# pirovc/ganon

Measured on AMD Instinct MI355X. Metric: Mreads/s classified (150 bp) + IBF-lookup GB/s vs HBM roofline, higher is better.
Workload: dtype u64

## Files before the change

ganon_amd/csrc/gn_kernels.hip:

```cpp
#include "gn_internal.h"
#include <cstdlib>

#define GN_WAVE 64
#define GN_CAND_LIMIT 128u
#ifndef GN_NARROW_MAX
#define GN_NARROW_MAX 4u
#endif
#include "gn_stray_probe.h"
static_assert(GN_PROBE_HASHES % 2u == 0 && GN_PROBE_HASHES * 4u <= GN_WAVE, "whole screen iterations (two hashes each), and stage 1 is one load a lane");
#define GN_MATCH_CHUNK 256u
#ifndef GN_MATCH_CHUNK_MAX
#define GN_MATCH_CHUNK_MAX 8192u
#endif
#define GN_STAGE_CAP 128u

struct GnRankLut
{
    uint8_t t[256];
    constexpr GnRankLut() : t{}
    {
        for (int i = 0; i < 256; ++i)
            t[i] = 0;
        t['C'] = t['c'] = 1;
        t['G'] = t['g'] = 2;
// ... 1434 lines not shown
                        q_to    = n;
                    }
                    const uint32_t inc  = add << (8u * (bit >> 3));
                    const uint32_t keep = SCR && finish ? ~(0xFFu << (8u * (bit >> 3))) : 0xFFFFFFFFu;
#pragma unroll
                    for (int j = 0; j < 4; ++j)
#pragma unroll
                        for (int pp = 0; pp < 2; ++pp)
                            if ((bit & 3u) == (uint32_t)j && ((bit >> 2) & 1u) == (uint32_t)pp && lane == L)
                                byt[d][j][pp] = (byt[d][j][pp] & keep) + inc;
                }
            }
        }
    }
    if (slice * 64 * LW < p.W)
    {
        const uint32_t wcol = p.W - slice * 64 * LW < 64u * LW ? p.W - slice * 64 * LW : 64u * LW;
        if constexpr (!SCR)
        {
            if (dead || narrow)
            {
                const uint32_t got  = fetched < n ? fetched : n;
                const uint64_t full = (uint64_t)(n - got) * HF * wcol * 8ull;
                const uint64_t part = (uint64_t)narrow_loads * 128ull;
                skipped_bytes += full - part;
            }
        }
        else if (dead || narrow || finish)
        {
            const uint32_t got  = fetched < n ? fetched : n;
            const uint32_t rows = SCR && scr_rows && !aborted ? scr_rows : got * HF;
            const uint64_t full = (uint64_t)(n * HF - rows) * wcol * 8ull;
            const uint64_t part = (uint64_t)narrow_loads * 128ull;
            skipped_bytes += full - part;
        }
        if (SCR && aborted)
            skipped_bytes -= (uint64_t)scr_rows * wcol * 8ull;
    }

    if (more)
        load_hashes(n_n, slot_n, hA_n, hB_n);

    uint32_t Kc  = (0x80u - T) * 0x01010101u;
    uint32_t any = 0;
    if (!dead)
    {
        if (acc_n)
            spill_nibbles();
#pragma unroll
        for (int d = 0; d < ND; ++d)
#pragma unroll
            for (int j = 0; j < 4; ++j)
#pragma unroll
                for (int pp = 0; pp < 2; ++pp)
                {
                    uint32_t x = byt[d][j][pp];
                    for (uint32_t off = Gp; off < GN_WAVE; off <<= 1)
                        x += __shfl_xor(x, (int)off);
                    byt[d][j][pp] = x;
                    any |= (x + Kc) & 0x80808080u;
                }
    }
    const bool owner = hsub == 0 && col_act;
    uint64_t   hm    = dead ? 0ull : __ballot(owner && any != 0);
    if (p.pre_mode && __popcll(hm) > 6)
    {
        auto any_ge = [&](uint32_t v) -> bool {
            const uint32_t K = (0x80u - v) * 0x01010101u;
            uint32_t       a = 0;
#pragma unroll
            for (int d = 0; d < ND; ++d)
#pragma unroll
                for (int j = 0; j < 4; ++j)
#pragma unroll
                    for (int pp = 0; pp < 2; ++pp)
                        a |= byt[d][j][pp] + K;
            return __ballot(owner && (a & 0x80808080u) != 0) != 0;
        };
        uint32_t lo = T, hi = n;
        while (lo < hi)
        {
            const uint32_t mid = (lo + hi + 1) >> 1;
            if (any_ge(mid))
                lo = mid;
            else
                hi = mid - 1;
        }
        const uint32_t t2 = gn_pf_threshold(lo, p.pre_mode == 1 ? T : 0u, p.pre_rel);
        if (t2 > T && t2 <= lo)
        {
            const uint32_t K2 = (0x80u - t2) * 0x01010101u;
            auto in_range = [&](uint32_t v, bool count) -> uint32_t {
                const uint32_t K1 = (0x80u - (v + 1u)) * 0x01010101u;
                uint32_t       a = 0;
#pragma unroll
                for (int d = 0; d < ND; ++d)
#pragma unroll
                    for (int j = 0; j < 4; ++j)
#pragma unroll
                        for (int pp = 0; pp < 2; ++pp)
                        {
                            const uint32_t e = ((byt[d][j][pp] + Kc) & ~(byt[d][j][pp] + K1)) & 0x80808080u;
                            a = count ? a + (uint32_t)__popc(e) : (a | e);
                        }
                return a;
            };
            const uint32_t below = owner ? in_range(t2 - 1u, true) : 0u;
            if (__ballot(below != 0))
            {
                uint32_t a = T, b = t2 - 1u;
                while (a < b)
                {
                    const uint32_t mid = (a + b) >> 1;
                    if (__ballot(owner && in_range(mid, false) != 0))
                        b = mid;
                    else
                        a = mid + 1u;
                }
                if (lane == 0)
                    p.seg_min[(size_t)read * wpr + slice] = a;
                n_pre += below;
                Kc  = K2;
                any = 0;
#pragma unroll
                for (int d = 0; d < ND; ++d)
#pragma unroll
                    for (int j = 0; j < 4; ++j)
#pragma unroll
                        for (int pp = 0; pp < 2; ++pp)
                            any |= (byt[d][j][pp] + Kc) & 0x80808080u;
                hm = __ballot(owner && any != 0);
            }
        }
    }
    uint32_t       total = 0;
    unsigned long long base = 0;
    if (hm)
    {
        uint32_t hit[ND];
        uint32_t mine = 0;
#pragma unroll
        for (int d = 0; d < ND; ++d)
        {
            hit[d] = 0;
            if (owner && any)
            {
#pragma unroll
                for (int j = 0; j < 4; ++j)
#pragma unroll
                    for (int pp = 0; pp < 2; ++pp)
                        hit[d] |= ((((byt[d][j][pp] + Kc) & 0x80808080u) >> 7) << (4 * pp + j));
            }
            mine += __popc(hit[d]);
        }
        uint32_t my_off = 0;
        if (__popcll(hm) <= 6)
        {
            uint64_t rem = hm;
            while (rem)
            {
                const uint32_t L = (uint32_t)__builtin_ctzll(rem);
                rem &= rem - 1;
                const uint32_t c = (uint32_t)__builtin_amdgcn_readlane((int)mine, (int)L);
                if ((uint32_t)lane == L)
                    my_off = total;
                total += c;
            }
        }
        else
        {
            uint32_t x = mine;
#pragma unroll
            for (int off = 1; off < GN_WAVE; off <<= 1)
            {
                const uint32_t y = (uint32_t)__shfl_up((int)x, off);
                if (lane >= off)
                    x += y;
            }
            my_off = x - mine;
            total  = (uint32_t)__builtin_amdgcn_readlane((int)x, GN_WAVE - 1);
        }
        if (total > chunk_left)
        {
            const uint32_t need = total > chunk_size ? total : chunk_size;
                chunk_size = chunk_size * 2u <= GN_MATCH_CHUNK_MAX ? chunk_size * 2u : GN_MATCH_CHUNK_MAX;
            unsigned long long nb = 0;
            if (lane == 0)
                nb = atomicAdd(p.cursor, (unsigned long long)need);
            chunk_base = gn_readlane64(nb, 0);
            chunk_left = need;
        }
        base = chunk_base;
        chunk_base += total;
        chunk_left -= total;
        const bool fits = base + total <= p.match_cap;
        if (__popcll(hm) > 6)
        {
            const uint8_t* tabb   = reinterpret_cast<const uint8_t*>(rowtab);
            const bool     listed = total <= GN_FAST_LIST;
            if (p.emit_probe & 128u)
                goto emitted;
            gn_match*      out    = p.matches + base + my_off;
            uint32_t       k      = 0;
#pragma unroll
            for (int d = 0; d < ND; ++d)
            {
                gn_wave_lds_sync();
                if (owner && any)
                {
#pragma unroll
                    for (int j = 0; j < 4; ++j)
#pragma unroll
                        for (int pp = 0; pp < 2; ++pp)
                            rowtab[(uint32_t)lane * 8u + (uint32_t)(j * 2 + pp)] = byt[d][j][pp];
                }
                gn_wave_lds_sync();
                uint32_t mbits = (fits && owner && any) ? hit[d] : 0u;
                while (mbits)
                {
                    const uint32_t b = (uint32_t)__builtin_ctz(mbits);
                    mbits &= mbits - 1;
                    const uint32_t cnt = tabb[(uint32_t)lane * 32u + (((b & 3u) << 1) + ((b >> 2) & 1u)) * 4u + (b >> 3)];
                    const uint32_t bin = (uint32_t)(gl * LW) * 64u + 32u * (uint32_t)d + b;
                    if (listed)
                        mlist[my_off + k] = (bin << 8) | cnt;
                    else
                    {
                        gn_match mt;
                        mt.read   = read;
                        mt.target = slice * 64u * LW * 64u + bin;
                        mt.count  = cnt;
                        out[k]    = mt;
                    }
                    ++k;
                }
            }
            gn_wave_lds_sync();
            if (listed && fits && !(p.emit_probe & 64u))
            {
                gn_match* seg = p.matches + base;
                for (uint32_t m = (uint32_t)lane; m < total; m += GN_WAVE)
                {
                    const uint32_t e = mlist[m];
                    gn_match       mt;
                    mt.read   = read;
                    mt.target = slice * 64u * LW * 64u + (e >> 8);
                    mt.count  = e & 0xFFu;
                    seg[m] = mt;
                }
                gn_wave_lds_sync();
            }
        }
        else if (fits && owner && any)
        {
            gn_match* out = p.matches + base + my_off;
            uint32_t  before = 0;
#pragma unroll
            for (int d = 0; d < ND; ++d)
            {
#pragma unroll
                for (int j = 0; j < 4; ++j)
#pragma unroll
                    for (int pp = 0; pp < 2; ++pp)
                    {
                        uint32_t hbits = (byt[d][j][pp] + Kc) & 0x80808080u;
                        while (hbits)
                        {
                            const uint32_t y = (uint32_t)__builtin_ctz(hbits) >> 3;
                            hbits &= hbits - 1;
                            const uint32_t bitpos = 8 * y + 4 * pp + j;
                            gn_match mt;
                            mt.read   = read;
                            mt.target = wi * 64 + 32 * d + bitpos;
                            mt.count  = (byt[d][j][pp] >> (8 * y)) & 0xFFu;
                            out[before + __popc(hit[d] & ((1u << bitpos) - 1u))] = mt;
                        }
                    }
                before += __popc(hit[d]);
            }
        }
    }
emitted:
    if (lane == 0)
    {
        p.seg_begin[(size_t)read * wpr + slice] = base;
        p.seg_count[(size_t)read * wpr + slice] = total;
    }
    if (!more)
        break;
    unit = unit_n; read = read_n; n = n_n; slot = slot_n; hA = hA_n; hB = hB_n;
    }
    if (lane == 0 && skipped_bytes)
        atomicAdd(p.skip_ctr, (unsigned long long)skipped_bytes);
    if (p.pre_mode)
    {
#pragma unroll
        for (int off = 32; off > 0; off >>= 1)
            n_pre += (uint32_t)__shfl_xor((int)n_pre, off);
        if (lane == 0 && n_pre)
            atomicAdd(p.pre_ctr, (unsigned long long)n_pre);
    }
}

#ifndef GN_FAST_WPE_LEAN
#define GN_FAST_WPE_LEAN 5
#endif
__global__ __launch_bounds__(256) __attribute__((amdgpu_waves_per_eu(GN_FAST_WPE_LEAN))) void gn_ibf_count_fast_kernel_lean(GnCountParams p)
{
    extern __shared__ __attribute__((aligned(16))) uint32_t gn_lds[];
    constexpr int      HF   = 4;
    constexpr int      ND   = 2;
    constexpr uint32_t NMAX = 127;

    const int      lane   = threadIdx.x & (GN_WAVE - 1);
    const int      wave   = __builtin_amdgcn_readfirstlane((int)(threadIdx.x >> 6));
    const uint32_t wpr    = p.wpr;
    uint32_t*      rowtab = gn_lds + (size_t)wave * 128 * HF;
    uint32_t*      pmask  = gn_lds + (size_t)(blockDim.x >> 6) * 128 * HF + (size_t)wave * (GN_PROBE_HASHES * ND * GN_WAVE);

    const uint64_t n_units = (uint64_t)(p.n_reads - p.read_begin) * wpr;
    const uint64_t stride  = (uint64_t)gridDim.x * (blockDim.x >> 6);
    uint64_t       unit    = (uint64_t)blockIdx.x * (blockDim.x >> 6) + wave;
    if (unit >= n_units)
        return;
    const bool     dyn      = p.grab != nullptr && n_units >= 64u * stride;
    const uint64_t dyn_from = stride * 16u;
    uint64_t       chunk_end = unit + 1;
    if (dyn)
    {
        unit *= 16u;
        chunk_end = unit + 16u;
    }
    unsigned long long g_next = 0;
    uint32_t           g_size = 16u;
    auto               ask    = [&](uint64_t from) {
        g_size = from < n_units - n_units / 4u ? 16u : (from < n_units - n_units / 16u ? 8u : 4u);
        if (lane == 0)
            g_next = atomicAdd(p.grab, (unsigned long long)g_size);
    };
    if (dyn)
        ask(unit);
    auto hash_of = [&](uint32_t& q0, uint32_t& q1) {
        uint32_t l = (uint32_t)lane;
        asm volatile("" : "+v"(l));
        q0 = l / HF;
        q1 = (l + GN_WAVE) / HF;
    };
    auto load_meta = [&](uint64_t u, uint32_t& rd, uint32_t& nn, uint64_t& so) {
        uint32_t w = wpr;
        asm volatile("" : "+s"(w));
        rd = p.read_begin + (uint32_t)(u / w);
        const uint32_t nh = p.n_hashes[rd];
        nn = p.status[rd] == GN_READ_OK ? nh : 0u;
        so = p.slot_off[rd];
    };
    auto load_hashes = [&](uint32_t nn, uint64_t so, uint64_t& h0, uint64_t& h1) {
        h0 = h1 = 0;
        if (nn >= 1 && nn <= NMAX)
        {
            uint32_t q0, q1;
            hash_of(q0, q1);
            if (q0 < nn)
                h0 = p.hashes[so + q0];
            if (q1 < nn)
                h1 = p.hashes[so + q1];
        }
    };
    unsigned long long chunk_base = 0;
    uint32_t           chunk_left = 0, chunk_size = GN_MATCH_CHUNK;
    uint64_t           skipped_bytes = 0;
    uint32_t read, n;
    uint64_t slot, hA, hB;
    load_meta(unit, read, n, slot);
    load_hashes(n, slot, hA, hB);

    for (;;)
    {
    const uint32_t slice = (uint32_t)(unit - (uint64_t)(read - p.read_begin) * wpr);
    uint64_t unit_n = unit + 1;
    if (unit_n >= chunk_end)
    {
        if (dyn)
        {
            const uint32_t lo32 = (uint32_t)__builtin_amdgcn_readfirstlane((int)(uint32_t)g_next);
            const uint32_t hi32 = (uint32_t)__builtin_amdgcn_readfirstlane((int)(uint32_t)(g_next >> 32));
            unit_n              = dyn_from + (((uint64_t)hi32 << 32) | lo32);
            chunk_end           = unit_n + g_size;
            if (unit_n < n_units)
                ask(unit_n);
        }
        else
        {
            unit_n    = unit + stride;
            chunk_end = unit_n + 1;
        }
    }
    const bool more = unit_n < n_units;
    uint32_t   read_n = 0, n_n = 0;
    uint64_t   slot_n = 0, hA_n = 0, hB_n = 0;

    const bool skip = n > NMAX || n == 0;
    uint32_t   T = 0, ds = 0;
    if (!skip)
    {
        T = (uint32_t)(uint64_t)ceil(__dmul_rn((double)n, p.rel_cutoff));
        if (T == 0)
            T = 1;
        if (p.early_exit && T >= 2)
        {
            ds = (p.screen[n >> 2] >> (8u * (n & 3u))) & 0xFFu;
            if (ds > n || ds + T <= n)
                ds = 0;
        }
    }
    if (skip || ds == 0)
    {
        if (lane == 0)
        {
            if (skip)
            {
                if (n > NMAX && slice == 0)
                    p.work_list_out[atomicAdd(p.work_count_out, 1ULL)] = read;
                uint32_t zero = 0;
                asm volatile("" : "+v"(zero));
                p.seg_begin[(size_t)read * wpr + slice] = zero;
                p.seg_count[(size_t)read * wpr + slice] = zero;
            }
            else
                p.unit_list_out[atomicAdd(p.unit_count_out, 1ULL)] = (uint32_t)unit;
        }
        if (!more)
            break;
        load_meta(unit_n, read_n, n_n, slot_n);
        load_hashes(n_n, slot_n, hA_n, hB_n);
        unit = unit_n; read = read_n; n = n_n; slot = slot_n; hA = hA_n; hB = hB_n;
        continue;
    }
    const uint32_t wi      = slice * 64 + (uint32_t)lane;
    const bool     col_act = wi < p.W;

    gn_wave_lds_sync();
    {
        uint32_t q0, q1;
        hash_of(q0, q1);
        if ((uint32_t)lane < n * HF)
            rowtab[(uint32_t)lane] = gn_ibf_row(hA, (uint32_t)lane - q0 * HF, p.shift, p.S);
        if ((uint32_t)lane + GN_WAVE < n * HF)
            rowtab[(uint32_t)lane + GN_WAVE] = gn_ibf_row(hB, (uint32_t)lane + GN_WAVE - q1 * HF, p.shift, p.S);
        for (uint32_t idx = (uint32_t)lane + 2 * GN_WAVE; idx < n * HF; idx += GN_WAVE)
        {
            const uint32_t q = idx / HF, i = idx - q * HF;
            rowtab[idx] = gn_ibf_row(p.hashes[slot + q], i, p.shift, p.S);
        }
    }
    gn_wave_lds_sync();

    uint32_t nib[ND][4];
    uint32_t byt[ND][4][2];
#pragma unroll
    for (int d = 0; d < ND; ++d)
#pragma unroll
        for (int j = 0; j < 4; ++j)
        {
            nib[d][j]    = 0;
            byt[d][j][0] = 0;
            byt[d][j][1] = 0;
        }
    uint32_t acc_n = 0;
    auto spill_nibbles = [&]() {
#pragma unroll
        for (int d = 0; d < ND; ++d)
#pragma unroll
            for (int j = 0; j < 4; ++j)
            {
                byt[d][j][0] += nib[d][j] & 0x0F0F0F0Fu;
                byt[d][j][1] += (nib[d][j] >> 4) & 0x0F0F0F0Fu;
                nib[d][j] = 0;
            }
    };
    const uint32_t wi_ld = col_act ? wi : 0u;
    auto issue = [&](uint32_t it, GnRowRegs<HF, 1>& R) {
        uint32_t row[HF];
#pragma unroll
        for (int i = 0; i < HF; ++i)
        {
            const uint32_t qs = 2 * it + (uint32_t)(i >> 1) < ds ? 2 * it + (uint32_t)(i >> 1) : 2 * it;
            row[i]            = rowtab[qs * HF + (uint32_t)(i & 1)];
        }
#pragma unroll
        for (int i = 0; i < HF; ++i)
        {
            const uint2 v = *reinterpret_cast<const uint2*>(p.rows + ((uint64_t)row[i] * p.W + wi_ld));
            R.m[i][0] = v.x;
            R.m[i][1] = v.y;
        }
    };
    auto consume = [&](const GnRowRegs<HF, 1>& R, uint32_t it) {
        const uint32_t on = col_act ? 0xFFFFFFFFu : 0u, on2 = 2 * it + 1 < ds ? on : 0u;
#pragma unroll
        for (int d = 0; d < ND; ++d)
        {
            const uint32_t a = R.m[0][d] & R.m[1][d] & on, b = R.m[2][d] & R.m[3][d] & on2;
            if (2 * it < GN_PROBE_HASHES)
            {
                uint32_t l = (uint32_t)lane;
                asm volatile("" : "+v"(l));
                pmask[((2 * it) * ND + (uint32_t)d) * GN_WAVE + l]     = a;
                pmask[((2 * it + 1) * ND + (uint32_t)d) * GN_WAVE + l] = b;
            }
#pragma unroll
            for (int j = 0; j < 4; ++j)
                nib[d][j] += ((a >> j) & 0x11111111u) + ((b >> j) & 0x11111111u);
        }
        acc_n += 2;
        if (acc_n >= 14)
        {
            spill_nibbles();
            acc_n = 0;
        }
    };
    GnRowRegs<HF, 1> A, Bq;
    issue(0, A);
    if (more)
        load_meta(unit_n, read_n, n_n, slot_n);
    {
        const uint32_t its = (ds + 1) >> 1;
        uint32_t       it  = 0;
        for (; it + 2 < its; it += 2)
        {
            issue(it + 1, Bq);
            consume(A, it);
            issue(it + 2, A);
            consume(Bq, it + 1);
        }
        const bool two = it + 1 < its;
        if (two)
            issue(it + 1, Bq);
        consume(A, it);
        if (two)
            consume(Bq, it + 1);
    }
    if (acc_n)
        spill_nibbles();
    uint32_t sm[ND];
    uint32_t left = 0;
    {
        const uint32_t Kt    = (0x80u - (T - (n - ds))) * 0x01010101u;
        uint32_t       any_t = 0;
#pragma unroll
        for (int d = 0; d < ND; ++d)
        {
            uint32_t m = 0;
#pragma unroll
            for (int j = 0; j < 4; ++j)
#pragma unroll
                for (int pp = 0; pp < 2; ++pp)
                {
                    const uint32_t g = (byt[d][j][pp] + Kt) & 0x80808080u;
                    any_t |= g;
                    m |= (g >> 7) << (4 * pp + j);
                }
            sm[d] = m;
        }
        if (__ballot(any_t != 0) != 0)
        {
            uint32_t c = 0;
#pragma unroll
            for (int d = 0; d < ND; ++d)
                c += (uint32_t)__popc(sm[d]);
            for (int off = 32; off > 0; off >>= 1)
                c += __shfl_xor(c, off);
            left = (uint32_t)__builtin_amdgcn_readfirstlane((int)c);
        }
    }
    const uint32_t wcol = slice * 64 < p.W ? (p.W - slice * 64 < 64u ? p.W - slice * 64 : 64u) : 0u;
    if (more)
        load_hashes(n_n, slot_n, hA_n, hB_n);
    if (left > GN_NARROW_MAX)
    {
        if (lane == 0)
            p.unit_list_out[atomicAdd(p.unit_count_out, 1ULL)] = (uint32_t)unit;
        skipped_bytes -= (uint64_t)(2 * ds) * wcol * 8ull;
        if (!more)
            break;
        unit = unit_n; read = read_n; n = n_n; slot = slot_n; hA = hA_n; hB = hB_n;
        continue;
    }
    uint32_t narrow_loads = 0;
    uint32_t total = 0;
    uint32_t rec_t = 0, rec_c = 0;
    if (left)
    {
        constexpr uint32_t QPC = GN_WAVE / HF;
        uint64_t           grp = 0;
#pragma unroll
        for (uint32_t q = 0; q < QPC; ++q)
            grp |= 1ULL << (q * HF);
        const uint32_t l_q = (uint32_t)lane / HF, l_i = (uint32_t)lane - l_q * HF;
        const uint32_t n_f = n, ds_f = ds;
        gn_wave_lds_sync();
        uint64_t       lm  = __ballot((sm[0] | sm[1]) != 0);
        while (lm)
        {
            const int L = __builtin_ctzll(lm);
            lm &= lm - 1;
#pragma unroll
            for (int d = 0; d < ND; ++d)
            {
                uint32_t mb = (uint32_t)__builtin_amdgcn_readlane((int)sm[d], L);
                while (mb)
                {
                    const uint32_t bit = (uint32_t)__builtin_ctz(mb);
                    mb &= mb - 1;
                    const uint32_t word = slice * 64 + (uint32_t)L;
                    const uint32_t sh   = 32u * d + bit;
                    uint32_t       c2   = 0;
#pragma unroll
                    for (int j = 0; j < 4; ++j)
#pragma unroll
                        for (int pp = 0; pp < 2; ++pp)
                            if ((bit & 3u) == (uint32_t)j && ((bit >> 2) & 1u) == (uint32_t)pp)
                                c2 = byt[d][j][pp];
                    c2 = ((uint32_t)__builtin_amdgcn_readlane((int)c2, L) >> (8u * (bit >> 3))) & 0xFFu;
                    uint32_t add     = 0;
                    uint32_t q_lo    = 0;
                    uint32_t q_known = ds_f;
                    uint32_t q_to    = n_f;
                    bool     probe   = c2 != ds;
                    bool     dropped = false;
                    uint32_t e1      = 0;
                    if (probe)
                    {
                        const uint32_t Fp   = gn_probe_first(p.probe_hashes, ds);
                        bool           hitq = false;
                        if (l_q < Fp)
                            hitq = ((pmask[(l_q * ND + (uint32_t)d) * GN_WAVE + (uint32_t)L] >> bit) & 1u) != 0;
                        const bool ld = hitq && l_i >= 2;
                        uint64_t   w1 = 0;
                        if (ld)
                            w1 = p.rows[(uint64_t)rowtab[l_q * HF + l_i] * p.W + word];
                        const uint64_t hb = __ballot(ld && ((w1 >> sh) & 1ULL));
                        const uint32_t m  = (uint32_t)__popcll(__ballot(hitq && l_i == 2));
                        e1                = (uint32_t)__popcll(hb & (hb >> 1) & (grp << 2));
                        narrow_loads += 2 * m;
                        dropped = gn_probe_drop1(n, T, ds, c2, m, e1);
                        q_lo    = Fp;
                        q_to    = ds_f;
                    }
                    while (!dropped)
                    {
                        add = 0;
                        for (uint32_t q0 = q_lo; q0 < q_to; q0 += 2 * QPC)
                        {
                            const uint32_t qa = q0 + l_q, qb = qa + QPC;
                            const bool     ina = qa < q_to, inb = qb < q_to;
                            uint64_t       wa = ~0ULL, wb = ~0ULL;
                            if (ina && !(l_i < 2 && qa < q_known))
                                wa = p.rows[(uint64_t)rowtab[qa * HF + l_i] * p.W + word];
                            if (inb && !(l_i < 2 && qb < q_known))
                                wb = p.rows[(uint64_t)rowtab[qb * HF + l_i] * p.W + word];
                            const uint64_t bma = __ballot(ina && ((wa >> sh) & 1ULL)), bmb = __ballot(inb && ((wb >> sh) & 1ULL));
                            uint64_t       alla = bma, allb = bmb;
#pragma unroll
                            for (int i = 1; i < HF; ++i)
                            {
                                alla &= bma >> i;
                                allb &= bmb >> i;
                            }
                            add += (uint32_t)__popcll(alla & grp) + (uint32_t)__popcll(allb & grp);
                        }
                        narrow_loads += (q_to - q_lo) * HF - 2 * (q_known - (probe ? q_lo : 0u));
                        if (!probe)
                            break;
                        probe = false;
                        add += e1;
                        if (gn_probe_drop2(n, T, ds, add))
                        {
                            add = 0;
                            break;
                        }
                        q_known = 0;
                        q_lo    = 0;
                        q_to    = n_f;
                    }
                    if (add >= T)
                    {
                        if ((uint32_t)lane == total)
                        {
                            rec_t = word * 64u + sh;
                            rec_c = add;
                        }
                        ++total;
                    }
                }
            }
        }
    }
    if (wcol)
        skipped_bytes += (uint64_t)(n * HF - 2 * ds) * wcol * 8ull - (uint64_t)narrow_loads * 128ull;

    unsigned long long base = 0;
    if (total)
    {
        if (total > chunk_left)
        {
            const uint32_t need = total > chunk_size ? total : chunk_size;
            chunk_size = chunk_size * 2u <= GN_MATCH_CHUNK_MAX ? chunk_size * 2u : GN_MATCH_CHUNK_MAX;
            unsigned long long nb = 0;
            if (lane == 0)
                nb = atomicAdd(p.cursor, (unsigned long long)need);
            chunk_base = gn_readlane64(nb, 0);
            chunk_left = need;
        }
        base = chunk_base;
        chunk_base += total;
        chunk_left -= total;
        uint32_t l = (uint32_t)lane;
        asm volatile("" : "+v"(l));
        if (base + total <= p.match_cap && l < total)
        {
            gn_match mt;
            mt.read   = read;
            mt.target = rec_t;
            mt.count  = rec_c;
            p.matches[base + l] = mt;
        }
    }
    if (lane == 0)
    {
        p.seg_begin[(size_t)read * wpr + slice] = base;
        p.seg_count[(size_t)read * wpr + slice] = total;
    }
    if (!more)
        break;
    unit = unit_n; read = read_n; n = n_n; slot = slot_n; hA = hA_n; hB = hB_n;
    }
    if (lane == 0 && skipped_bytes)
        atomicAdd(p.skip_ctr, (unsigned long long)skipped_bytes);
}

template <int HF, int LW, int MAXT>
static hipError_t gn_launch_count_one(const GnCountParams& p, const GnCountGeometry& g, hipStream_t st)
{
    uint32_t blocks = (p.n_reads - p.read_begin + g.rpb - 1) / g.rpb;
    if (blocks > p.max_blocks)
        blocks = p.max_blocks;
    (void)hipFuncSetAttribute(reinterpret_cast<const void*>(gn_ibf_count_kernel<HF, LW, MAXT>),
                              hipFuncAttributeMaxDynamicSharedMemorySize, (int)g.lds_bytes);
    hipLaunchKernelGGL((gn_ibf_count_kernel<HF, LW, MAXT>), dim3(blocks), dim3(g.block), g.lds_bytes, st, p);
    return hipGetLastError();
}

template <int HF, int LW>
static hipError_t gn_launch_fast_one(const GnCountParams& p, hipStream_t st)
{
    const bool ee = p.early_exit && p.gp_log2 == GN_FAST_EE_GP_LOG2;
    const uint64_t units  = (uint64_t)(p.n_reads - p.read_begin) * p.wpr;
    uint32_t       blocks = (uint32_t)((units + 3) / 4);
    if (blocks > p.max_blocks_fast)
        blocks = p.max_blocks_fast;
    const size_t   lds    = 4 * (128 * (HF <= 4 ? 4 : 8) + GN_FAST_LIST) * 4;
    const size_t   lds_pm = 4 * (GN_PROBE_HASHES * 2 * LW * GN_WAVE) * 4;
    bool scr = false;
    if constexpr (HF == 4)
        for (uint32_t w : p.screen)
            scr = scr || w != 0;
    scr = scr && ee;
    if constexpr (HF == 4 && LW == 2)
        if (scr && p.W > 128)
        {
            hipLaunchKernelGGL((gn_ibf_count_fast_kernel<HF, LW, true, true, true>), dim3(blocks), dim3(256), lds + lds_pm, st, p);
            return hipGetLastError();
        }
    if constexpr (HF == 4 && LW == 1)
        if (scr && p.unit_list_out != nullptr)
        {
            uint32_t lean_blocks = (uint32_t)((units + 3) / 4);
            if (lean_blocks > p.max_blocks_lean)
                lean_blocks = p.max_blocks_lean;
            hipLaunchKernelGGL(gn_ibf_count_fast_kernel_lean, dim3(lean_blocks), dim3(256), 4 * (128 * HF + GN_PROBE_HASHES * 2 * GN_WAVE) * 4, st, p);
            hipError_t e = hipGetLastError();
            if (e != hipSuccess)
                return e;
            GnCountParams q = p;
            q.unit_list     = p.unit_list_out;
            q.unit_count    = p.unit_count_out;
            q.grab          = nullptr;
            if (blocks > p.max_blocks_list)
                blocks = p.max_blocks_list;
            hipLaunchKernelGGL((gn_ibf_count_fast_kernel<HF, LW, true>), dim3(blocks ? blocks : 1u), dim3(256), lds, st, q);
            return hipGetLastError();
        }
    if constexpr (HF == 4 && LW == 1)
        if (scr)
        {
            hipLaunchKernelGGL((gn_ibf_count_fast_kernel<HF, LW, true, false, true>), dim3(blocks), dim3(256), lds + lds_pm, st, p);
            return hipGetLastError();
        }
    if (ee && LW == 2 && p.W > 128)
        hipLaunchKernelGGL((gn_ibf_count_fast_kernel<HF, LW, true, LW == 2>), dim3(blocks), dim3(256), lds, st, p);
    else if (ee)
        hipLaunchKernelGGL((gn_ibf_count_fast_kernel<HF, LW, true>), dim3(blocks), dim3(256), lds, st, p);
    else
        hipLaunchKernelGGL((gn_ibf_count_fast_kernel<HF, LW, false>), dim3(blocks), dim3(256), lds, st, p);
    return hipGetLastError();
}

hipError_t gn_launch_count_fast(const GnCountParams& p, const GnCountGeometry& g, uint32_t hash_funs, hipStream_t st)
{
    if (p.n_reads <= p.read_begin)
        return hipSuccess;
    const bool two = g.lw == 2;
    switch (hash_funs)
    {
        case 1: return two ? gn_launch_fast_one<1, 2>(p, st) : gn_launch_fast_one<1, 1>(p, st);
        case 2: return two ? gn_launch_fast_one<2, 2>(p, st) : gn_launch_fast_one<2, 1>(p, st);
        case 3: return two ? gn_launch_fast_one<3, 2>(p, st) : gn_launch_fast_one<3, 1>(p, st);
        case 4: return two ? gn_launch_fast_one<4, 2>(p, st) : gn_launch_fast_one<4, 1>(p, st);
        case 5: return two ? gn_launch_fast_one<5, 2>(p, st) : gn_launch_fast_one<5, 1>(p, st);
        default: return hipErrorInvalidValue;
    }
}

template <int HF>
static hipError_t gn_launch_count_hf(const GnCountParams& p, const GnCountGeometry& g, hipStream_t st)
{
    if (g.block <= 256)
        return g.lw == 2 ? gn_launch_count_one<HF, 2, 256>(p, g, st) : gn_launch_count_one<HF, 1, 256>(p, g, st);
    if (g.block <= 512)
        return g.lw == 2 ? gn_launch_count_one<HF, 2, 512>(p, g, st) : gn_launch_count_one<HF, 1, 512>(p, g, st);
    return g.lw == 2 ? gn_launch_count_one<HF, 2, 1024>(p, g, st) : gn_launch_count_one<HF, 1, 1024>(p, g, st);
}

hipError_t gn_launch_count(const GnCountParams& p, const GnCountGeometry& g, uint32_t hash_funs, hipStream_t st)
{
    if (p.n_reads <= p.read_begin)
        return hipSuccess;
    switch (hash_funs)
    {
        case 1: return gn_launch_count_hf<1>(p, g, st);
        case 2: return gn_launch_count_hf<2>(p, g, st);
        case 3: return gn_launch_count_hf<3>(p, g, st);
        case 4: return gn_launch_count_hf<4>(p, g, st);
        case 5: return gn_launch_count_hf<5>(p, g, st);
        default: return hipErrorInvalidValue;
    }
}

__global__ void gn_long_list_kernel(const uint8_t* __restrict__ status, uint32_t read_begin, uint32_t n_reads,
                                    uint32_t* __restrict__ list, unsigned long long* __restrict__ count)
{
    const uint32_t r = read_begin + blockIdx.x * blockDim.x + threadIdx.x;
    if (r < n_reads && status[r] == GN_READ_BIG)
        list[atomicAdd(count, 1ULL)] = r;
}

__global__ __launch_bounds__(256) void gn_ibf_count_long_kernel(GnCountParams p, uint32_t* __restrict__ scratch)
{
    __shared__ uint32_t           part[256];
    __shared__ unsigned long long base_sh;
    __shared__ uint32_t           total_sh;
    const uint32_t tid   = threadIdx.x;
    uint32_t*      cnt   = scratch + (size_t)blockIdx.x * ((size_t)p.B + 64);
    const uint32_t n_work = (uint32_t)*p.work_count;
    const uint32_t hf    = p.early_exit;
    for (uint32_t widx = blockIdx.x; widx < n_work; widx += gridDim.x)
    {
        const uint32_t read = p.work_list[widx];
        const uint32_t n    = p.n_hashes[read];
        for (uint32_t i = tid; i < p.B; i += 256)
            cnt[i] = 0;
        __syncthreads();
        const uint64_t* hs = p.hashes + p.slot_off[read];
        for (uint32_t q = 0; q < n; ++q)
        {
            const uint64_t v = hs[q];
            uint32_t       row[5];
            for (uint32_t i = 0; i < hf; ++i)
                row[i] = gn_ibf_row(v, i, p.shift, p.S);
            for (uint32_t j = tid; j < p.W; j += 256)
            {
                uint64_t m = p.rows[(uint64_t)row[0] * p.W + j];
                for (uint32_t i = 1; i < hf; ++i)
                    m &= p.rows[(uint64_t)row[i] * p.W + j];
                while (m)
                {
                    const uint32_t b = j * 64u + (uint32_t)__builtin_ctzll(m);
                    m &= m - 1;
                    if (b < p.B)
                        cnt[b]++;
                }
            }
        }
        __syncthreads();
        uint64_t T = (uint64_t)ceil(__dmul_rn((double)n, p.rel_cutoff));
        if (T == 0)
            T = 1;
        const uint32_t per = (p.n_targets + 255u) / 256u;
        const uint32_t lo  = tid * per < p.n_targets ? tid * per : p.n_targets;
        const uint32_t hi  = lo + per < p.n_targets ? lo + per : p.n_targets;
        auto           summed = [&](uint32_t t) -> uint64_t {
            uint64_t c = 0;
            if (!p.tgt_off)
                c = cnt[t];
            else
                for (uint32_t e = p.tgt_off[t]; e < p.tgt_off[t + 1]; ++e)
                    c += cnt[p.tgt_bins[e]];
            return c > n ? (uint64_t)n : c;
        };
        uint32_t mine = 0;
        for (uint32_t t = lo; t < hi; ++t)
            mine += summed(t) >= T ? 1u : 0u;
        part[tid] = mine;
        __syncthreads();
        if (tid == 0)
        {
            uint32_t run = 0;
            for (uint32_t i = 0; i < 256; ++i)
            {
                const uint32_t c = part[i];
                part[i]          = run;
                run += c;
            }
            base_sh = run ? atomicAdd(p.cursor, (unsigned long long)run) : 0ull;
            for (uint32_t sl = 0; sl < p.wpr; ++sl)
            {
                p.seg_begin[(size_t)read * p.wpr + sl] = sl == 0 ? base_sh : 0ull;
                p.seg_count[(size_t)read * p.wpr + sl] = sl == 0 ? run : 0u;
            }
            total_sh = run;
        }
        __syncthreads();
        const uint32_t           total = total_sh;
        const unsigned long long base  = base_sh;
        if (base + total <= p.match_cap)
        {
            uint32_t k = part[tid];
            for (uint32_t t = lo; t < hi; ++t)
            {
                const uint64_t c = summed(t);
                if (c >= T)
                {
                    gn_match mt;
                    mt.read   = read;
                    mt.target = p.tgt_ids ? p.tgt_ids[t] : t;
                    mt.count  = (uint32_t)c;
                    p.matches[base + k++] = mt;
                }
            }
        }
        __syncthreads();
    }
}

hipError_t gn_launch_count_long(const GnCountParams& p, uint32_t hash_funs, uint32_t* list, unsigned long long* count, uint32_t* scratch,
                                uint32_t blocks, hipStream_t st)
{
    const uint32_t n = p.n_reads - p.read_begin;
    if (n == 0)
        return hipSuccess;
    hipLaunchKernelGGL(gn_long_list_kernel, dim3((n + 255) / 256), dim3(256), 0, st, p.status, p.read_begin, p.n_reads, list, count);
    GnCountParams q = p;
    q.work_list  = list;
    q.work_count = count;
    q.early_exit = hash_funs;
    hipLaunchKernelGGL(gn_ibf_count_long_kernel, dim3(blocks), dim3(256), 0, st, q, scratch);
    return hipGetLastError();
}

__global__ void gn_emplace_kernel(uint64_t* rows, uint64_t S, uint32_t W, uint32_t shift, uint32_t h,
                                  const uint64_t* __restrict__ hashes, const uint32_t* __restrict__ bins, uint64_t n)
{
    const uint64_t idx = (uint64_t)blockIdx.x * blockDim.x + threadIdx.x;
    if (idx >= n * h)
        return;
    const uint64_t q   = idx / h;
    const uint32_t i   = (uint32_t)(idx - q * h);
    const uint32_t bin = bins[q];
    const uint32_t row = gn_ibf_row(hashes[q], i, shift, S);
    atomicOr(reinterpret_cast<unsigned long long*>(rows + ((uint64_t)row * W + (bin >> 6))), 1ULL << (bin & 63));
}

hipError_t gn_launch_emplace(uint64_t* rows, uint64_t S, uint32_t W, uint32_t shift, uint32_t h, const uint64_t* hashes,
                             const uint32_t* bins, uint64_t n, hipStream_t st)
{
    if (n == 0)
        return hipSuccess;
    const uint64_t total  = n * h;
    const uint32_t blocks = (uint32_t)((total + 255) / 256);
    hipLaunchKernelGGL(gn_emplace_kernel, dim3(blocks), dim3(256), 0, st, rows, S, W, shift, h, hashes, bins, n);
    return hipGetLastError();
}
```

Measured before the change: 305.1.

## Double-buffer row tables and prime next unit's first loads in lean count kernel

The lean IBF count kernel now keeps two per-wave row tables in LDS. It builds the next unit's row indices and issues that unit's first row loads (prime) before the current unit finishes its narrow/probe stage, so hashing and the first memory latency overlap with the current work. The row hash is specialised for four hash functions to cut index arithmetic. The cost is doubled row-table LDS per block, which may lower occupancy, plus extra register pressure from carrying T/ds and the prefetched registers across iterations.

```diff
diff --git a/ganon_amd/csrc/gn_kernels.hip b/ganon_amd/csrc/gn_kernels.hip
--- a/ganon_amd/csrc/gn_kernels.hip
+++ b/ganon_amd/csrc/gn_kernels.hip
@@ -1760,6 +1760,15 @@
     }
 }
 
+__device__ __forceinline__ uint32_t gn_ibf_row4(uint64_t v, uint32_t i, uint32_t shift, uint64_t S)
+{
+    constexpr uint64_t seeds[GN_IBF_MAX_HASH_FUNS] = GN_IBF_SEED_LIST;
+    const uint64_t     lo = (i & 1u) ? seeds[1] : seeds[0], hi = (i & 1u) ? seeds[3] : seeds[2];
+    uint64_t           x  = v * ((i & 2u) ? hi : lo);
+    x ^= x >> shift;
+    x *= GN_IBF_MULTIPLIER;
+    return (uint32_t)__umul64hi(x, S);
+}
 #ifndef GN_FAST_WPE_LEAN
 #define GN_FAST_WPE_LEAN 5
 #endif
@@ -1773,8 +1782,9 @@
     const int      lane   = threadIdx.x & (GN_WAVE - 1);
     const int      wave   = __builtin_amdgcn_readfirstlane((int)(threadIdx.x >> 6));
     const uint32_t wpr    = p.wpr;
-    uint32_t*      rowtab = gn_lds + (size_t)wave * 128 * HF;
-    uint32_t*      pmask  = gn_lds + (size_t)(blockDim.x >> 6) * 128 * HF + (size_t)wave * (GN_PROBE_HASHES * ND * GN_WAVE);
+    constexpr uint32_t TABW = 128 * HF;
+    uint32_t*      rowtab = gn_lds + (size_t)wave * 2 * TABW;
+    uint32_t*      pmask  = gn_lds + (size_t)(blockDim.x >> 6) * 2 * TABW + (size_t)wave * (GN_PROBE_HASHES * ND * GN_WAVE);
 
     const uint64_t n_units = (uint64_t)(p.n_reads - p.read_begin) * wpr;
     const uint64_t stride  = (uint64_t)gridDim.x * (blockDim.x >> 6);
@@ -1827,10 +1837,68 @@
     unsigned long long chunk_base = 0;
     uint32_t           chunk_left = 0, chunk_size = GN_MATCH_CHUNK;
     uint64_t           skipped_bytes = 0;
-    uint32_t read, n;
-    uint64_t slot, hA, hB;
-    load_meta(unit, read, n, slot);
-    load_hashes(n, slot, hA, hB);
+    auto plan = [&](uint32_t nn, uint32_t& T_, uint32_t& ds_) {
+        T_ = 0;
+        ds_ = 0;
+        if (nn >= 1 && nn <= NMAX)
+        {
+            T_ = (uint32_t)(uint64_t)ceil(__dmul_rn((double)nn, p.rel_cutoff));
+            if (T_ == 0)
+                T_ = 1;
+            if (p.early_exit && T_ >= 2)
+            {
+                ds_ = (p.screen[nn >> 2] >> (8u * (nn & 3u))) & 0xFFu;
+                if (ds_ > nn || ds_ + T_ <= nn)
+                    ds_ = 0;
+            }
+        }
+    };
+    auto issue = [&](const uint32_t* tb, uint32_t dsv, uint32_t wld, uint32_t it, GnRowRegs<HF, 1>& R) {
+        uint32_t row[HF];
+#pragma unroll
+        for (int i = 0; i < HF; ++i)
+        {
+            const uint32_t qs = 2 * it + (uint32_t)(i >> 1) < dsv ? 2 * it + (uint32_t)(i >> 1) : 2 * it;
+            row[i]            = tb[qs * HF + (uint32_t)(i & 1)];
+        }
+#pragma unroll
+        for (int i = 0; i < HF; ++i)
+        {
+            const uint2 v = *reinterpret_cast<const uint2*>(p.rows + ((uint64_t)row[i] * p.W + wld));
+            R.m[i][0] = v.x;
+            R.m[i][1] = v.y;
+        }
+    };
+    GnRowRegs<HF, 1> A, Bq;
+    auto prime = [&](uint64_t un, uint32_t& rd, uint32_t& nn, uint64_t so, uint64_t h0, uint64_t h1, uint32_t* tb, uint32_t& T_, uint32_t& ds_) {
+        rd = (uint32_t)__builtin_amdgcn_readfirstlane((int)rd);
+        nn = (uint32_t)__builtin_amdgcn_readfirstlane((int)nn);
+        plan(nn, T_, ds_);
+        T_  = (uint32_t)__builtin_amdgcn_readfirstlane((int)T_);
+        ds_ = (uint32_t)__builtin_amdgcn_readfirstlane((int)ds_);
+        if (ds_ == 0)
+            return;
+        gn_wave_lds_sync();
+        uint32_t l = (uint32_t)lane;
+        asm volatile("" : "+v"(l));
+        if (l < nn * HF)
+            tb[l] = gn_ibf_row4(h0, l % HF, p.shift, p.S);
+        if (l + GN_WAVE < nn * HF)
+            tb[l + GN_WAVE] = gn_ibf_row4(h1, l % HF, p.shift, p.S);
+        for (uint32_t idx = l + 2 * GN_WAVE; idx < nn * HF; idx += GN_WAVE)
+            tb[idx] = gn_ibf_row4(p.hashes[so + idx / HF], idx % HF, p.shift, p.S);
+        gn_wave_lds_sync();
+        const uint32_t w = (uint32_t)(un - (uint64_t)(rd - p.read_begin) * wpr) * 64 + l;
+        issue(tb, ds_, w < p.W ? w : 0u, 0, A);
+    };
+    uint32_t read, n, T, ds;
+    uint32_t tab = 0;
+    {
+        uint64_t slot, h0, h1;
+        load_meta(unit, read, n, slot);
+        load_hashes(n, slot, h0, h1);
+        prime(unit, read, n, slot, h0, h1, rowtab, T, ds);
+    }
 
     for (;;)
     {
@@ -1854,23 +1922,11 @@
         }
     }
     const bool more = unit_n < n_units;
-    uint32_t   read_n = 0, n_n = 0;
+    uint32_t   read_n = 0, n_n = 0, T_n = 0, ds_n = 0;
     uint64_t   slot_n = 0, hA_n = 0, hB_n = 0;
+    uint32_t*  tab_n = rowtab + (tab ^ TABW);
 
     const bool skip = n > NMAX || n == 0;
-    uint32_t   T = 0, ds = 0;
-    if (!skip)
-    {
-        T = (uint32_t)(uint64_t)ceil(__dmul_rn((double)n, p.rel_cutoff));
-        if (T == 0)
-            T = 1;
-        if (p.early_exit && T >= 2)
-        {
-            ds = (p.screen[n >> 2] >> (8u * (n & 3u))) & 0xFFu;
-            if (ds > n || ds + T <= n)
-                ds = 0;
-        }
-    }
     if (skip || ds == 0)
     {
         if (lane == 0)
@@ -1891,26 +1947,14 @@
             break;
         load_meta(unit_n, read_n, n_n, slot_n);
         load_hashes(n_n, slot_n, hA_n, hB_n);
-        unit = unit_n; read = read_n; n = n_n; slot = slot_n; hA = hA_n; hB = hB_n;
+        prime(unit_n, read_n, n_n, slot_n, hA_n, hB_n, tab_n, T_n, ds_n);
+        unit = unit_n; read = read_n; n = n_n; T = T_n; ds = ds_n; tab ^= TABW;
         continue;
     }
-    const uint32_t wi      = slice * 64 + (uint32_t)lane;
-    const bool     col_act = wi < p.W;
-
-    gn_wave_lds_sync();
-    {
-        uint32_t q0, q1;
-        hash_of(q0, q1);
-        if ((uint32_t)lane < n * HF)
-            rowtab[(uint32_t)lane] = gn_ibf_row(hA, (uint32_t)lane - q0 * HF, p.shift, p.S);
-        if ((uint32_t)lane + GN_WAVE < n * HF)
-            rowtab[(uint32_t)lane + GN_WAVE] = gn_ibf_row(hB, (uint32_t)lane + GN_WAVE - q1 * HF, p.shift, p.S);
-        for (uint32_t idx = (uint32_t)lane + 2 * GN_WAVE; idx < n * HF; idx += GN_WAVE)
-        {
-            const uint32_t q = idx / HF, i = idx - q * HF;
-            rowtab[idx] = gn_ibf_row(p.hashes[slot + q], i, p.shift, p.S);
-        }
-    }
+    const uint32_t  wi      = slice * 64 + (uint32_t)lane;
+    const bool      col_act = wi < p.W;
+    const uint32_t* tab_c   = rowtab + tab;
+
     gn_wave_lds_sync();
 
     uint32_t nib[ND][4];
@@ -1937,22 +1981,6 @@
             }
     };
     const uint32_t wi_ld = col_act ? wi : 0u;
-    auto issue = [&](uint32_t it, GnRowRegs<HF, 1>& R) {
-        uint32_t row[HF];
-#pragma unroll
-        for (int i = 0; i < HF; ++i)
-        {
-            const uint32_t qs = 2 * it + (uint32_t)(i >> 1) < ds ? 2 * it + (uint32_t)(i >> 1) : 2 * it;
-            row[i]            = rowtab[qs * HF + (uint32_t)(i & 1)];
-        }
-#pragma unroll
-        for (int i = 0; i < HF; ++i)
-        {
-            const uint2 v = *reinterpret_cast<const uint2*>(p.rows + ((uint64_t)row[i] * p.W + wi_ld));
-            R.m[i][0] = v.x;
-            R.m[i][1] = v.y;
-        }
-    };
     auto consume = [&](const GnRowRegs<HF, 1>& R, uint32_t it) {
         const uint32_t on = col_act ? 0xFFFFFFFFu : 0u, on2 = 2 * it + 1 < ds ? on : 0u;
 #pragma unroll
@@ -1977,8 +2005,6 @@
             acc_n = 0;
         }
     };
-    GnRowRegs<HF, 1> A, Bq;
-    issue(0, A);
     if (more)
         load_meta(unit_n, read_n, n_n, slot_n);
     {
@@ -1986,14 +2012,16 @@
         uint32_t       it  = 0;
         for (; it + 2 < its; it += 2)
         {
-            issue(it + 1, Bq);
+            issue(tab_c, ds, wi_ld, it + 1, Bq);
             consume(A, it);
-            issue(it + 2, A);
+            issue(tab_c, ds, wi_ld, it + 2, A);
             consume(Bq, it + 1);
         }
         const bool two = it + 1 < its;
         if (two)
-            issue(it + 1, Bq);
+            issue(tab_c, ds, wi_ld, it + 1, Bq);
+        if (more)
+            load_hashes(n_n, slot_n, hA_n, hB_n);
         consume(A, it);
         if (two)
             consume(Bq, it + 1);
@@ -2033,7 +2061,7 @@
     }
     const uint32_t wcol = slice * 64 < p.W ? (p.W - slice * 64 < 64u ? p.W - slice * 64 : 64u) : 0u;
     if (more)
-        load_hashes(n_n, slot_n, hA_n, hB_n);
+        prime(unit_n, read_n, n_n, slot_n, hA_n, hB_n, tab_n, T_n, ds_n);
     if (left > GN_NARROW_MAX)
     {
         if (lane == 0)
@@ -2041,7 +2069,7 @@
         skipped_bytes -= (uint64_t)(2 * ds) * wcol * 8ull;
         if (!more)
             break;
-        unit = unit_n; read = read_n; n = n_n; slot = slot_n; hA = hA_n; hB = hB_n;
+        unit = unit_n; read = read_n; n = n_n; T = T_n; ds = ds_n; tab ^= TABW;
         continue;
     }
     uint32_t narrow_loads = 0;
@@ -2054,7 +2082,9 @@
 #pragma unroll
         for (uint32_t q = 0; q < QPC; ++q)
             grp |= 1ULL << (q * HF);
-        const uint32_t l_q = (uint32_t)lane / HF, l_i = (uint32_t)lane - l_q * HF;
+        uint32_t l_f = (uint32_t)lane;
+        asm volatile("" : "+v"(l_f));
+        const uint32_t l_q = l_f / HF, l_i = l_f - l_q * HF;
         const uint32_t n_f = n, ds_f = ds;
         gn_wave_lds_sync();
         uint64_t       lm  = __ballot((sm[0] | sm[1]) != 0);
@@ -2096,7 +2126,7 @@
                         const bool ld = hitq && l_i >= 2;
                         uint64_t   w1 = 0;
                         if (ld)
-                            w1 = p.rows[(uint64_t)rowtab[l_q * HF + l_i] * p.W + word];
+                            w1 = p.rows[(uint64_t)tab_c[l_q * HF + l_i] * p.W + word];
                         const uint64_t hb = __ballot(ld && ((w1 >> sh) & 1ULL));
                         const uint32_t m  = (uint32_t)__popcll(__ballot(hitq && l_i == 2));
                         e1                = (uint32_t)__popcll(hb & (hb >> 1) & (grp << 2));
@@ -2114,9 +2144,9 @@
                             const bool     ina = qa < q_to, inb = qb < q_to;
                             uint64_t       wa = ~0ULL, wb = ~0ULL;
                             if (ina && !(l_i < 2 && qa < q_known))
-                                wa = p.rows[(uint64_t)rowtab[qa * HF + l_i] * p.W + word];
+                                wa = p.rows[(uint64_t)tab_c[qa * HF + l_i] * p.W + word];
                             if (inb && !(l_i < 2 && qb < q_known))
-                                wb = p.rows[(uint64_t)rowtab[qb * HF + l_i] * p.W + word];
+                                wb = p.rows[(uint64_t)tab_c[qb * HF + l_i] * p.W + word];
                             const uint64_t bma = __ballot(ina && ((wa >> sh) & 1ULL)), bmb = __ballot(inb && ((wb >> sh) & 1ULL));
                             uint64_t       alla = bma, allb = bmb;
 #pragma unroll
@@ -2191,7 +2221,7 @@
     }
     if (!more)
         break;
-    unit = unit_n; read = read_n; n = n_n; slot = slot_n; hA = hA_n; hB = hB_n;
+    unit = unit_n; read = read_n; n = n_n; T = T_n; ds = ds_n; tab ^= TABW;
     }
     if (lane == 0 && skipped_bytes)
         atomicAdd(p.skip_ctr, (unsigned long long)skipped_bytes);
@@ -2236,7 +2266,7 @@
             uint32_t lean_blocks = (uint32_t)((units + 3) / 4);
             if (lean_blocks > p.max_blocks_lean)
                 lean_blocks = p.max_blocks_lean;
-            hipLaunchKernelGGL(gn_ibf_count_fast_kernel_lean, dim3(lean_blocks), dim3(256), 4 * (128 * HF + GN_PROBE_HASHES * 2 * GN_WAVE) * 4, st, p);
+            hipLaunchKernelGGL(gn_ibf_count_fast_kernel_lean, dim3(lean_blocks), dim3(256), 4 * (2 * 128 * HF + GN_PROBE_HASHES * 2 * GN_WAVE) * 4, st, p);
             hipError_t e = hipGetLastError();
             if (e != hipSuccess)
                 return e;
```

Result: slower. 285.8 (-6.3%).
